# Desperodoo/distributed_multi_agent_reinforcement_learning

Hardware: AMD Instinct MI355X
Metric: env-steps/sec (whole node), pursuit-evasion 8-agent 4096-env (higher is better)
Workload: dtype f64 environment / f32 policy (f32 matrix products evaluated from exact 3-way bf16 operand splits, f32 accumulation and storage)

## Files before the change

distributed_multi_agent_reinforcement_learning_amd/csrc/mappo_split.hip:

```cpp
#include <hip/hip_runtime.h>
#include <stdint.h>
#include <string.h>

#include "mappo_ops.h"
#include "sb_gemm.hpp"
#include "sb_encoder_tail.hpp"
#include "sb_gru_seq.hpp"

extern "C" {

static int sb_gemm_any(int64_t R, int32_t N, int32_t K, const float *X, int64_t ldx, const float *W, int64_t ldw, const float *bias, int32_t relu,
                       const float *addend, int64_t lda, float *Y, int64_t ldy, uint8_t *ybits, int64_t ldyb, void *stream) {
    if (R < 0 || !X || !W || !Y || ldx < K || ldw < K || ldy < N || (addend && lda < N)) return MO_ERR_BAD_ARG;
    if ((ldx & 3) || (ldw & 3) || (ldy & 3) || (lda & 3) || ((uintptr_t)X & 15) || ((uintptr_t)W & 15) || ((uintptr_t)Y & 15) || ((uintptr_t)addend & 15) ||
        ((uintptr_t)bias & 15))
        return MO_ERR_BAD_ARG;
    if (R == 0) return 0;
    hipStream_t st = (hipStream_t)stream;
    if (N == 128 && K == 128) return launch_sb_gemm_best<4, 1>(R, X, ldx, W, ldw, bias, addend, lda, Y, ldy, relu, st, ybits, ldyb);
    if (N == 128 && K == 256) return launch_sb_gemm_best<8, 1>(R, X, ldx, W, ldw, bias, addend, lda, Y, ldy, relu, st, ybits, ldyb);
    if (ybits) return MO_ERR_BAD_ARG;
    if (N == 128 && K == 384) return launch_sb_gemm_best<12, 1>(R, X, ldx, W, ldw, bias, addend, lda, Y, ldy, relu, st);
    if (N == 256 && K == 128) return launch_sb_gemm_best<4, 2>(R, X, ldx, W, ldw, bias, addend, lda, Y, ldy, relu, st);
    if (N == 384 && K == 128) return launch_sb_gemm_best<4, 3>(R, X, ldx, W, ldw, bias, addend, lda, Y, ldy, relu, st);
    return MO_ERR_BAD_ARG;
}

int sb_gemm(int64_t R, int32_t N, int32_t K, const float *X, int64_t ldx, const float *W, int64_t ldw, const float *bias, int32_t relu,
            const float *addend, int64_t lda, float *Y, int64_t ldy, void *stream) {
// ... 41 lines not shown
    if (hipGetDevice(&dev) == hipSuccess && hipDeviceGetAttribute(&cus, hipDeviceAttributeMultiprocessorCount, dev) != hipSuccess) cus = 256;
    if (cus > 512) return MO_ERR_BAD_ARG;
    float *part = (float *)workspace;
    const float *m = (const float *)sign_bits;
    const int mt = mask_cols / 128;
    if (N == 256 && K == 128) return launch_sb_gemm<4, 2, SBG_MASK_OPT_256 | 16>(R, X, ldx, W, ldw, nullptr, m, ld_bytes, Y, ldy, 0, st, mt, part, colsum);
    if (N == 384 && K == 128) return launch_sb_gemm<4, 3, SBG_MASK_OPT_384 | 16>(R, X, ldx, W, ldw, nullptr, m, ld_bytes, Y, ldy, 0, st, mt, part, colsum);
    if (N == 128 && K == 384) return launch_sb_gemm<12, 1, SBG_MASK_OPT_K384 | 16>(R, X, ldx, W, ldw, nullptr, m, ld_bytes, Y, ldy, 0, st, mt, part, colsum);
    return MO_ERR_BAD_ARG;
}

int sb_gemm_n128(int64_t R, int32_t K, const float *X, int64_t ldx, const float *W, int64_t ldw, const float *bias, int32_t relu, const float *addend,
                 int64_t lda, float *Y, int64_t ldy, void *stream) {
    return sb_gemm(R, 128, K, X, ldx, W, ldw, bias, relu, addend, lda, Y, ldy, stream);
}

int sb_encoder_tail(int64_t Rs, const float *m3, int64_t ldx, const float *w_agg, const float *b_agg, const float *Ws, int64_t ldw, const float *C,
                    int64_t ldc, float *Y, int64_t ldy, void *stream) {
    if (Rs < 0 || !m3 || !w_agg || !b_agg || !Ws || !C || !Y || ldx < 384 || ldw < 384 || ldc < 128 || ldy < 128) return MO_ERR_BAD_ARG;
    if ((ldx & 3) || (ldw & 3) || (ldc & 3) || (ldy & 3) || ((uintptr_t)m3 & 15) || ((uintptr_t)w_agg & 15) || ((uintptr_t)b_agg & 15) || ((uintptr_t)Ws & 15) ||
        ((uintptr_t)C & 15) || ((uintptr_t)Y & 15))
        return MO_ERR_BAD_ARG;
    if (Rs == 0) return 0;
    return launch_sb_encoder_tail(Rs, m3, ldx, w_agg, b_agg, Ws, ldw, C, ldc, Y, ldy, (hipStream_t)stream);
}

int gru_seq_split_fwd_multi(int32_t n_nets, const mo_gru_seq_net *nets, int32_t T, int32_t B, int32_t H, int32_t gi_agents, void *stream) {
    if (n_nets < 1 || n_nets > MO_GRU_MAX_NETS || !nets || T < 1 || B < 1 || H != SBR_H || gi_agents < 0 || (gi_agents && B % gi_agents)) return MO_ERR_BAD_ARG;
    for (int k = 0; k < n_nets; k++) {
        const mo_gru_seq_net &m = nets[k];
        if (!m.gi || !m.w_hh || !m.b_hh || !m.h0 || !m.out) return MO_ERR_BAD_ARG;
        if ((((uintptr_t)m.gi | (uintptr_t)m.w_hh | (uintptr_t)m.b_hh | (uintptr_t)m.h0 | (uintptr_t)m.out | (uintptr_t)m.save) & 15)) return MO_ERR_BAD_ARG;
        if (m.B < 0 || m.B > B || (gi_agents && m.B % gi_agents)) return MO_ERR_BAD_ARG;
    }
    return launch_gru_seq_fwd_sb(n_nets, nets, T, B, gi_agents, (hipStream_t)stream);
}

int gru_seq_split_bwd_multi(int32_t n_nets, const mo_gru_seq_bwd_net *nets, int32_t T, int32_t B, int32_t H, int32_t gi_agents, void *stream) {
    if (n_nets < 1 || n_nets > MO_GRU_MAX_NETS || !nets || T < 1 || B < 1 || H != SBR_H || gi_agents < 0 || (gi_agents && B % gi_agents)) return MO_ERR_BAD_ARG;
    for (int k = 0; k < n_nets; k++) {
        const mo_gru_seq_bwd_net &m = nets[k];
        if (!m.dout || !m.save || !m.out || !m.h0 || !m.w_hh || !m.dgi || !m.dh0) return MO_ERR_BAD_ARG;
        if ((m.dgh == nullptr) == (m.dnr == nullptr)) return MO_ERR_BAD_ARG;
        if ((m.db_ih || m.db_hh) && (!m.db_ih || !m.db_hh || !m.workspace)) return MO_ERR_BAD_ARG;
        if ((((uintptr_t)m.dout | (uintptr_t)m.save | (uintptr_t)m.out | (uintptr_t)m.h0 | (uintptr_t)m.dgi | (uintptr_t)m.dgh | (uintptr_t)m.dnr |
              (uintptr_t)m.dh0 | (uintptr_t)m.workspace) & 15)) return MO_ERR_BAD_ARG;
        if (m.B < 0 || m.B > B || (gi_agents && m.B % gi_agents)) return MO_ERR_BAD_ARG;
// ... 6 lines not shown
```

distributed_multi_agent_reinforcement_learning_amd/csrc/sb_encoder_tail.hpp:

```cpp
#pragma once
#include <mutex>

#include "sb_common.hpp"

constexpr int SBE_IMG = 3 * 4 * 2 * 64;
constexpr int SBE_WIMG = 8 * 4 * 3 * 64;

__global__ __launch_bounds__(512) void k_sb_encoder_tail(int64_t Rs, const float *__restrict__ X, int64_t ldx, const float *__restrict__ Wa,
                                                         const float *__restrict__ ba, const float *__restrict__ Ws, int64_t ldw, const float *C,
                                                         int64_t ldc, float *Y, int64_t ldy) {
    extern __shared__ uint4 sbe_lds[];
    const int tid = threadIdx.x, w = tid >> 6, l = tid & 63, i = l & 15, gq = l >> 4;
    uint4 *const wimg = sbe_lds + w * (4 * 3 * 64) + l, *const mimg = sbe_lds + SBE_WIMG, *const eimg = mimg + SBE_IMG;
    {
        const float *rw = Wa + (size_t)(16 * w + i) * 128 + 8 * gq;
#pragma unroll
        for (int c = 0; c < 4; c++) {
            uint4 p_[3];
            sb_split8(*(const float4 *)(rw + 32 * c), *(const float4 *)(rw + 32 * c + 4), p_);
#pragma unroll
            for (int p = 0; p < 3; p++) wimg[(c * 3 + p) * 64] = p_[p];
        }
    }
    uint4 ws[12][3];
    {
        const float *rw = Ws + (size_t)(16 * w + i) * ldw + 8 * gq;
#pragma unroll
        for (int c = 0; c < 12; c++) sb_split8(*(const float4 *)(rw + 32 * c), *(const float4 *)(rw + 32 * c + 4), ws[c]);
    }
    const float4 b4 = *(const float4 *)(ba + 16 * w + 4 * gq);
    const int64_t n_t = (Rs + 31) / 32, G = gridDim.x;
    float4 pf[2];
    auto fetch = [&](int64_t t, int r) {
        const int64_t row = t * 32 + (w & 1) * 16 + i;
        pf[0] = pf[1] = make_float4(0.f, 0.f, 0.f, 0.f);
        if (row < Rs) {
            const float *src = X + row * ldx + 128 * r + 32 * (w >> 1) + 8 * gq;
            pf[0] = *(const float4 *)src;
            pf[1] = *(const float4 *)(src + 4);
        }
    };
    auto stage = [&]() {
        uint4 p_[3];
        sb_split8(pf[0], pf[1], p_);
#pragma unroll
        for (int p = 0; p < 3; p++) mimg[(p * 8 + w) * 64 + l] = p_[p];
    };
    uint2 *const edst = (uint2 *)eimg + (((w >> 1) * 2) * 64 + ((2 * (w & 1) + (gq >> 1)) << 4) + i) * 2 + (gq & 1);
    int64_t t = blockIdx.x;
    if (t < n_t) { fetch(t, 0); stage(); fetch(t, 1); }
    lds_barrier();
    for (; t < n_t; t += G) {
        const bool more = t + G < n_t;
        float4 a4[2];
#pragma unroll
        for (int rt = 0; rt < 2; rt++) {
            const int64_t row = t * 32 + rt * 16 + i;
            a4[rt] = row < Rs ? *(const float4 *)(C + row * ldc + 16 * w + 4 * gq) : make_float4(0.f, 0.f, 0.f, 0.f);
        }
        f32x4 acc_s[2];
        acc_s[0] = acc_s[1] = (f32x4){0.f, 0.f, 0.f, 0.f};
#pragma unroll
        for (int r = 0; r < 3; r++) {
            f32x4 acc_a[2];
            acc_a[0] = acc_a[1] = (f32x4){0.f, 0.f, 0.f, 0.f};
#define SBE_MMA(A, pi, pj)                                                                                                                          \
            acc[0] = __builtin_amdgcn_mfma_f32_16x16x32_bf16(__builtin_bit_cast(bf16x8, A[pi]), __builtin_bit_cast(bf16x8, b0[pj]), acc[0], 0, 0, 0); \
            acc[1] = __builtin_amdgcn_mfma_f32_16x16x32_bf16(__builtin_bit_cast(bf16x8, A[pi]), __builtin_bit_cast(bf16x8, b1[pj]), acc[1], 0, 0, 0);
#define SBE_MMA6(A) SBE_MMA(A, 2, 0) SBE_MMA(A, 0, 2) SBE_MMA(A, 1, 1) SBE_MMA(A, 1, 0) SBE_MMA(A, 0, 1) SBE_MMA(A, 0, 0)
#pragma unroll
            for (int c = 0; c < 4; c++) {
                uint4 a_[3], b0[3], b1[3];
#pragma unroll
                for (int p = 0; p < 3; p++) { a_[p] = wimg[(c * 3 + p) * 64]; b0[p] = mimg[(p * 8 + 2 * c) * 64 + l]; b1[p] = mimg[(p * 8 + 2 * c + 1) * 64 + l]; }
                f32x4(&acc)[2] = acc_a;
                SBE_MMA6(a_)
            }
#pragma unroll
            for (int rt = 0; rt < 2; rt++) {
                float4 v = make_float4(acc_a[rt][0] + b4.x, acc_a[rt][1] + b4.y, acc_a[rt][2] + b4.z, acc_a[rt][3] + b4.w);
                v.x = fmaxf(v.x, 0.f); v.y = fmaxf(v.y, 0.f); v.z = fmaxf(v.z, 0.f); v.w = fmaxf(v.w, 0.f);
                uint32_t lo[3], hi[3];
                sb_split2(v.x, v.y, lo[0], lo[1], lo[2]);
                sb_split2(v.z, v.w, hi[0], hi[1], hi[2]);
#pragma unroll
                for (int p = 0; p < 3; p++) edst[p * 8 * 64 * 2 + rt * 128] = make_uint2(lo[p], hi[p]);
            }
            lds_barrier();
            auto next_step = [&]() {
                if (r < 2 || more) stage();
                if (r == 0) fetch(t, 2);
                else if (more) fetch(t + G, r - 1);
            };
            if (w < 4) next_step();
#pragma unroll
            for (int c = 0; c < 4; c++) {
                uint4 b0[3], b1[3];
#pragma unroll
                for (int p = 0; p < 3; p++) { b0[p] = eimg[(p * 8 + 2 * c) * 64 + l]; b1[p] = eimg[(p * 8 + 2 * c + 1) * 64 + l]; }
                f32x4(&acc)[2] = acc_s;
                SBE_MMA6(ws[4 * r + c])
            }
#undef SBE_MMA6
#undef SBE_MMA
            if (w >= 4) next_step();
            if (r < 2) lds_barrier();
        }
#pragma unroll
        for (int rt = 0; rt < 2; rt++) {
            const int64_t row = t * 32 + rt * 16 + i;
            if (row < Rs) {
                float4 v = make_float4(acc_s[rt][0] + 0.f, acc_s[rt][1] + 0.f, acc_s[rt][2] + 0.f, acc_s[rt][3] + 0.f);
                v.x += a4[rt].x; v.y += a4[rt].y; v.z += a4[rt].z; v.w += a4[rt].w;
                *(float4 *)(Y + row * ldy + 16 * w + 4 * gq) = v;
            }
        }
        lds_barrier();
    }
}

inline int launch_sb_encoder_tail(int64_t Rs, const float *X, int64_t ldx, const float *Wa, const float *ba, const float *Ws, int64_t ldw,
                                  const float *C, int64_t ldc, float *Y, int64_t ldy, hipStream_t st) {
    constexpr int lds = (SBE_WIMG + 2 * SBE_IMG) * 16;
    static std::once_flag once;
    static hipError_t attr_rc = hipSuccess;
    std::call_once(once, [] { attr_rc = hipFuncSetAttribute((const void *)k_sb_encoder_tail, hipFuncAttributeMaxDynamicSharedMemorySize, lds); });
    if (attr_rc != hipSuccess) return (int)attr_rc;
    int dev = 0, cus = 256;
    if (hipGetDevice(&dev) == hipSuccess && hipDeviceGetAttribute(&cus, hipDeviceAttributeMultiprocessorCount, dev) != hipSuccess) cus = 256;
    const int64_t n_t = (Rs + 31) / 32;
    const int grid = n_t < (int64_t)cus ? (int)n_t : cus;
    hipLaunchKernelGGL(k_sb_encoder_tail, dim3(grid), dim3(512), lds, st, Rs, X, ldx, Wa, ba, Ws, ldw, C, ldc, Y, ldy);
    return (int)hipGetLastError();
}
```

distributed_multi_agent_reinforcement_learning_amd/model.py:

```python
import torch
import torch.nn as nn
import torch.nn.functional as F
from torch.nn.utils import spectral_norm
from torch.nn.utils.spectral_norm import SpectralNorm

from . import ops


class HeadLinear(nn.Linear):

    def forward(self, x):
        return ops.linear_skinny(x, self.weight, self.bias)


def _ortho_linear(n_in, n_out, cls=nn.Linear):
    layer = cls(n_in, n_out)
    for name, param in layer.named_parameters():
        if "bias" in name:
            nn.init.constant_(param, 0)
        elif "weight" in name:
            nn.init.orthogonal_(param, gain=1.0)
    return layer


# ... 17 lines not shown
        if self.num_relation != 3:
            raise NotImplementedError("num_relation must be 3 (defender, evader, obstacle)")
        self.input_dim, self.embedding_dim = input_dim, embedding_dim
        E = embedding_dim
        self.semantic_layer = _make_linear(3 * E + input_dim, E, is_sn)
        for r in range(self.num_relation):
            self.MSG_layers.append(_make_linear(2 * input_dim if r == 0 else input_dim, E, is_sn))
        for _ in range(self.depth):
            self.FCRA_layers.append(_make_linear(2 * E, E, is_sn))
        self.AGG_layers["AGG_vertex_0"] = _make_linear(E, E, is_sn)
        for k in range(self.depth):
            self.AGG_layers[f"AGG_fcra_{k}"] = _make_linear(E, E, is_sn)

    def encoder(self, p, e, o, adj_p, adj_e, adj_o, is_critic, o_kvalid=None, q_div=1, out=None, e_ref=None):
        M = self.MSG_layers
        m3 = ops.msg_agg3(p, e, o, adj_p, adj_e, adj_o, M[0].weight, M[0].bias, M[1].weight, M[1].bias, M[2].weight, M[2].bias,
                          is_critic, o_kvalid, q_div, e_ref)
        return self._after_messages(p, m3, out)

    def _after_messages(self, p, m3, out=None):
        R, P = p.shape[0], p.shape[1]
        E, ind = self.embedding_dim, self.input_dim
        agg0 = self.AGG_layers["AGG_vertex_0"]
        link = ops.ReluLink()
        emb = ops.linear(m3, agg0.weight, agg0.bias, relu=True, y_link=link)
        Ws = self.semantic_layer.weight
        p2, e2 = p.reshape(R * P, ind), emb.reshape(R * P, 3 * E)
        if out is not None:
            o2 = out.view(R * P, E)
            torch.addmm(self.semantic_layer.bias, p2, Ws[:, :ind].t(), out=o2)
            h0 = o2.addmm_(e2, Ws[:, ind:].t())
        else:
            h0 = ops.linear(e2, Ws[:, ind:], ops.linear_skinny(p2, Ws[:, :ind], self.semantic_layer.bias), consume_addend=True, x_link=link)
        return h0.reshape(R, P, E)

    def encoder_pair_train(self, p, e, o, adj_p, adj_e, adj_o, q_div=1, e_ref=None):
        M = self.MSG_layers
        m3a, m3c = ops.msg_agg3_pair_train(p, e, o, adj_p, adj_e, adj_o, M[0].weight, M[0].bias, M[1].weight, M[1].bias, M[2].weight, M[2].bias,
                                           q_div, e_ref)
        return self._after_messages(p, m3a), self._after_messages(p, m3c)

    def fcra(self, h0, hist, adj_p, is_critic, out=None):
        if self.depth == 0:
            return h0
        h, carry = h0, None
        for k in range(self.depth):
            aggk, fk = self.AGG_layers[f"AGG_fcra_{k}"], self.FCRA_layers[k]
            nb = ops.fcra_mean(z_critic=hist[k]) if is_critic else ops.fcra_mean(z_actor=hist[k], adj=adj_p)
            last = k == self.depth - 1
            h, carry = ops.fcra_hop(nb, h, carry, aggk.weight, aggk.bias, fk.weight, fk.bias, last, out if last else None)
        h.relu_link = carry[1]
        return h

    def forward(self, p, e, o, adj_p, adj_e, adj_o, hist, is_critic, o_kvalid=None, q_div=1, out=None, e_ref=None):
        h0 = self.encoder(p, e, o, adj_p, adj_e, adj_o, is_critic, o_kvalid, q_div, out if self.depth == 0 else None, e_ref)
        return self.fcra(h0, hist, adj_p, is_critic, out)
# ... 287 lines not shown
```

distributed_multi_agent_reinforcement_learning_amd/ops.py:

```python
import ctypes as C
import os

import torch
import torch.nn.functional as F

from . import build as _build

ADJ_TENSOR, ADJ_ONES, ADJ_VALID, ADJ_BITS = 0, 1, 2, 3
EXPORTS = ("dhgn_msg_agg_fwd", "dhgn_msg_agg3_fwd", "dhgn_msg_agg_bwd", "dhgn_msg_agg_bwd_workspace", "dhgn_msg_agg_ones_sorted_ok", "dhgn_msg_agg_ones_sorted_fwd",
           "dhgn_msg_agg_ones_sorted_bwd", "dhgn_msg_agg_ones_sorted_workspace", "gae_advnorm", "gae_advnorm_workspace", "categorical_sample",
           "categorical_sample_counter",
           "gru_gates_fwd", "gru_gates_bwd", "gru_cell_fwd", "gru_cell_fwd_multi", "gru_cell_split_fwd_multi", "sb_gemm_n128", "sb_gemm", "sb_encoder_tail", "gru_seq_fwd", "gru_seq_fwd_multi", "gru_seq_split_fwd_multi", "gru_seq_split_bwd_multi", "gru_seq_save_elems", "gru_seq_bwd", "gru_seq_bwd_multi", "gru_seq_bwd_workspace", "wgrad_tn", "wgrad_tn_workspace", "wgrad_split_tn", "wgrad_split_tn2", "wgrad_split_workspace", "rollout_record", "ppo_loss_fwd_bwd", "ppo_loss_prob_fwd_bwd", "ppo_loss_workspace",
           "gauss_head_sample", "ppo_loss_gauss_fwd_bwd", "ppo_loss_gauss_workspace", "gauss_head_sample_ex", "ppo_loss_gauss_ex_fwd_bwd",
           "ppo_loss_gauss_ex_workspace", "gae_advnorm_vn", "gae_advnorm_vn_workspace", "value_norm_update", "value_norm_targets",
           "ppo_loss_fwd_bwd_diag", "ppo_loss_prob_fwd_bwd_diag", "ppo_loss_gauss_fwd_bwd_diag", "ppo_loss_gauss_ex_fwd_bwd_diag",
           "ppo_loss_diag_workspace", "ppo_loss_gauss_diag_workspace", "ppo_ratio", "ppo_diag_rows_host", "fused_adam_workspace",
           "fused_adam_grid", "fused_adam_norm", "fused_adam_step", "fused_adam_advance_host", "fused_adam_rows_host", "bc_loss_workspace",
           "bc_loss_gauss_fwd_bwd", "bc_loss_gauss_ex_fwd_bwd", "bc_loss_cat_fwd_bwd", "e3d_bc_select", "n2n_bc_select", "ppo_bc_loss_workspace",
           "ppo_bc_loss_gauss_fwd_bwd", "ppo_bc_loss_cat_fwd_bwd", "mappo_ops_error_string")

_lib = None


def lib_path():
# ... 24 lines not shown
        L.dhgn_msg_agg_ones_sorted_workspace.restype = i64
        L.dhgn_msg_agg_ones_sorted_fwd.argtypes = [i32, i32, i32, i32, vp, i64, vp, i64, i32, vp, vp, vp, i64, vp, vp, vp]
        L.dhgn_msg_agg_ones_sorted_bwd.argtypes = [i32, i32, i32, i32, vp, i64, i32, vp, i64, vp, vp, vp, vp, vp, vp]
        L.gae_advnorm.argtypes = [i32, i32, i32, vp, vp, vp, f32, f32, i32, vp, vp, vp, vp]
        L.gae_advnorm_workspace.restype = i64
        L.gae_advnorm_vn.argtypes = [i32, i32, i32, vp, vp, vp, vp, vp, f32, f32, i32, vp, vp, vp, vp, vp]
        L.gae_advnorm_vn_workspace.restype = i64
        L.value_norm_update.argtypes = [vp, vp, C.c_double, vp]
        L.value_norm_targets.argtypes = [i64, vp, vp, vp, vp, vp]
        L.categorical_sample.argtypes = [i32, i32, vp, C.c_uint64, C.c_uint64, i32, vp, vp, vp]
        L.categorical_sample_counter.argtypes = [i32, i32, vp, C.c_uint64, vp, i32, vp, vp, vp]
        L.head_linear.argtypes = [i32, i32, i32, vp, vp, vp, vp, vp]
        L.head_sample.argtypes = [i32, i32, i32, vp, vp, vp, C.c_uint64, vp, vp, i32, vp, vp, vp]
        L.gru_gates_fwd.argtypes = [i32, i32, vp, vp, vp, vp, vp, vp, vp]
        L.gru_gates_bwd.argtypes = [i32, i32, vp, vp, vp, vp, vp, vp, vp, vp]
        L.gru_cell_fwd.argtypes = [i32, i32, vp, vp, vp, vp, vp, vp, vp, vp]
        L.gru_seq_fwd.argtypes = [i32, i32, i32, vp, vp, vp, vp, vp, vp, i32, vp]
        L.gru_seq_bwd.argtypes = [i32, i32, i32, vp, vp, vp, vp, vp, vp, vp, vp, vp, vp, vp, i32, vp, vp]
        L.gru_cell_fwd_multi.argtypes = [i32, vp, i32, i32, vp]
        L.gru_cell_split_fwd_multi.argtypes = [i32, vp, i32, i32, vp]
        L.sb_gemm_n128.argtypes = [i64, i32, vp, i64, vp, i64, vp, i32, vp, i64, vp, i64, vp]
        L.sb_gemm.argtypes = [i64, i32, i32, vp, i64, vp, i64, vp, i32, vp, i64, vp, i64, vp]
        L.sb_encoder_tail.argtypes = [i64, vp, i64, vp, vp, vp, i64, vp, i64, vp, i64, vp]
        L.gru_seq_fwd_multi.argtypes = [i32, vp, i32, i32, i32, i32, vp]
        L.gru_seq_bwd_multi.argtypes = [i32, vp, i32, i32, i32, i32, vp]
        L.gru_seq_split_fwd_multi.argtypes = [i32, vp, i32, i32, i32, i32, vp]
        L.gru_seq_split_bwd_multi.argtypes = [i32, vp, i32, i32, i32, i32, vp]
        L.gru_seq_save_elems.argtypes = [i32, i32]
        L.gru_seq_save_elems.restype = i64
        L.gru_seq_bwd_workspace.argtypes = [i32]
        L.gru_seq_bwd_workspace.restype = i64
        L.wgrad_tn_workspace.argtypes = [i32, i32]
        L.wgrad_tn_workspace.restype = i64
        L.wgrad_tn.argtypes = [i64, i32, i32, vp, i64, vp, i64, vp, i32, vp, vp]
        L.wgrad_split_workspace.restype = i64
        L.wgrad_split_workspace.argtypes = [i32, i32]
        L.wgrad_split_tn.argtypes = [i64, i32, i32, vp, i64, vp, i64, vp, i32, vp, vp]
        L.wgrad_split_tn2.argtypes = [i64, i32, i32, i32, vp, i64, vp, i64, vp, i64, vp, i32, vp, vp]
        L.fcra_neighbour_mean.argtypes = [i32, i32, i32, i32, vp, i64, i64, vp, i64, i64, vp, i64, vp, i32, vp, vp, i64, vp]
        L.fcra_neighbour_mean_multi.argtypes = [i32, vp, i32, i32, i32, i32, i64, i64, i64, i64, vp, i64, i32, i64, vp]
        L.sb_gemm_signs.argtypes = [i64, i32, i32, vp, i64, vp, i64, vp, i32, vp, i64, vp, i64, vp, i64, vp]
        L.sb_gemm_masked_bits.argtypes = [i64, i32, i32, vp, i64, vp, i64, vp, i64, i32, vp, i64, vp, vp, vp]
        L.sb_gemm_masked_workspace.argtypes = [i32]
        L.sb_gemm_masked_workspace.restype = i64
        L.sb_gemm_masked.argtypes = [i64, i32, i32, vp, i64, vp, i64, vp, i64, i32, vp, i64, vp, vp, vp]
        L.relu_bwd_colsum_workspace.argtypes = [i32]
# ... 1719 lines not shown
    if m3.dim() != 2 or out.dim() != 2 or m3.shape[1] != 384 or tuple(out.shape) != (m3.shape[0], 128) or tuple(Ws.shape) != (128, 384):
        return False
    if tuple(w_agg.shape) != (128, 128) or not w_agg.is_contiguous() or b_agg is None or tuple(b_agg.shape) != (128,) or not b_agg.is_contiguous():
        return False
    for t in (m3, w_agg, Ws, out):
        if t.dtype != torch.float32 or t.stride(1) != 1 or t.stride(0) % 4 or t.data_ptr() % 16:
            return False
    if b_agg.dtype != torch.float32 or b_agg.data_ptr() % 16:
        return False
    return not _overlap(m3, out)


def encoder_tail(m3, w_agg, b_agg, Ws, out):
    L = load_library()
    _check(L.sb_encoder_tail(m3.shape[0], _ptr(m3), m3.stride(0), _ptr(w_agg.detach()), _ptr(b_agg.detach()), _ptr(Ws.detach()), Ws.stride(0),
                             _ptr(out), out.stride(0), _ptr(out), out.stride(0), _stream()), "sb_encoder_tail")
    return out


def sign_bits_ok(N, K):
    return RELU_LINK and RELU_BITS and N == 128 and K in (128, 256)


PROJ_MODE = os.environ.get("MAPPO_PROJ", MATMUL_MODE)


def gru_input_projection(x2, w_ih, b_ih):
    if x2.stride(-1) == 1 and split_linear_ok(x2, w_ih, mode=PROJ_MODE, shapes=UPDATE_SPLIT_SHAPES):
        return split_linear(x2, w_ih, b_ih)
    return torch.addmm(b_ih, x2, w_ih.t())


def gru_step_multi(xs, hiddens, modules, hiddens_out=None):
    n = len(xs)
    B = xs[0].shape[0]
    outs_h = hiddens if hiddens_out is None else hiddens_out
    ok = (not torch.is_grad_enabled() and n <= 4 and B >= FUSED_CELL_MIN_ROWS and all(x.shape == (B, 128) and x.is_cuda for x in xs)
          and all(h.is_contiguous() and h.shape[1:] == (B, 128) for h in list(hiddens) + list(outs_h))
          and all(m.num_layers == modules[0].num_layers and m.weight_hh_l0.shape == (384, 128) and m.weight_ih_l0.shape == (384, 128) for m in modules))
    if not ok:
        outs = []
        for x, h, ho, m in zip(xs, hiddens, outs_h, modules):
            out, hn = gru(x.unsqueeze(0), h, m, inplace_hidden=hiddens_out is None)
            if hn is not ho:
                ho.copy_(hn)
            outs.append(ho[-1])
# ... 197 lines not shown
```

include/mappo_ops.h:

```cpp
#ifndef MAPPO_OPS_H
#define MAPPO_OPS_H
#include <stdint.h>

#ifdef __cplusplus
extern "C" {
#endif

#define MO_ERR_BAD_ARG 20001

enum { MO_ADJ_TENSOR = 0,
       MO_ADJ_ONES = 1,
       MO_ADJ_VALID = 2,
       MO_ADJ_BITS = 3 };
#define MO_ADJ_ROW_WORDS(K) (((((K) + 31) >> 5) + 3) & ~3)

int dhgn_msg_agg_fwd(int32_t R, int32_t P, int32_t K, int32_t E, int32_t din, const float *p, int64_t p_row_stride,
                     const float *q, int64_t q_row_stride, int32_t q_div, const float *e, int64_t e_row_stride, const void *adj,
                     int64_t adj_row_stride, int32_t adj_mode, const int32_t *kvalid, const float *W, const float *b,
                     float *out, int64_t out_stride , void *stream);

typedef struct mo_msg_rel {
    int32_t K, din, q_div, adj_mode;
    const float *q; int64_t q_rs;
    const float *e; int64_t e_rs;
// ... 88 lines not shown
int64_t gru_seq_bwd_workspace(int32_t B);
int gru_seq_bwd(int32_t T, int32_t B, int32_t H, const float *dout, const float *save, const float *out, const float *h0,
                const float *w_hh, float *dgi, float *dgh, float *dnr, float *dh0, float *db_ih, float *db_hh, int32_t gi_agents,
                void *workspace, void *stream);

int gru_cell_fwd(int32_t B, int32_t H, const float *x, const float *h_prev, const float *w_ih, const float *w_hh, const float *b_ih,
                 const float *b_hh, float *h_out, void *stream);
typedef struct mo_gru_cell_net { const float *x, *h_prev, *w_ih, *w_hh, *b_ih, *b_hh; float *h_out; } mo_gru_cell_net;
int gru_cell_fwd_multi(int32_t n_nets, const mo_gru_cell_net *nets, int32_t B, int32_t H, void *stream);
int gru_cell_split_fwd_multi(int32_t n_nets, const mo_gru_cell_net *nets, int32_t B, int32_t H, void *stream);
int sb_gemm_n128(int64_t R, int32_t K, const float *X, int64_t ldx, const float *W, int64_t ldw, const float *bias, int32_t relu, const float *C,
                 int64_t ldc, float *Y, int64_t ldy, void *stream);
int sb_gemm(int64_t R, int32_t N, int32_t K, const float *X, int64_t ldx, const float *W, int64_t ldw, const float *bias, int32_t relu, const float *C,
            int64_t ldc, float *Y, int64_t ldy, void *stream);
int sb_encoder_tail(int64_t Rs, const float *m3, int64_t ldx, const float *w_agg, const float *b_agg, const float *Ws, int64_t ldw, const float *C,
                    int64_t ldc, float *Y, int64_t ldy, void *stream);
int sb_gemm_signs(int64_t R, int32_t N, int32_t K, const float *X, int64_t ldx, const float *W, int64_t ldw, const float *bias, int32_t relu, const float *C,
                  int64_t ldc, float *Y, int64_t ldy, uint8_t *y_sign_bits, int64_t ld_bytes, void *stream);
int64_t sb_gemm_masked_workspace(int32_t N);
int sb_gemm_masked(int64_t R, int32_t N, int32_t K, const float *X, int64_t ldx, const float *W, int64_t ldw, const float *M, int64_t ldm,
                   int32_t mask_cols, float *Y, int64_t ldy, float *colsum, void *workspace, void *stream);
int sb_gemm_masked_bits(int64_t R, int32_t N, int32_t K, const float *X, int64_t ldx, const float *W, int64_t ldw, const uint8_t *sign_bits,
                        int64_t ld_bytes, int32_t mask_cols, float *Y, int64_t ldy, float *colsum, void *workspace, void *stream);

int64_t ppo_loss_workspace(void);
int ppo_loss_fwd_bwd(int64_t n, const float *logp_now, const float *entropy, const float *logp_old, const float *adv, const float *active,
                     const float *values_now, const float *values_old, const float *v_target, const float *active_sum, float epsilon,
                     float entropy_coef, int32_t use_value_clip, float *losses, float *grad_logp, float *grad_entropy, float *grad_values,
                     void *workspace, void *stream);
int ppo_loss_prob_fwd_bwd(int64_t n, int32_t A, const float *prob, float *grad_prob, int64_t d1, int64_t d2, int64_t p_s0, int64_t p_s1, int64_t p_s2,
                          const float *action, const float *logp_old, const float *adv, const float *active, const float *values_now, int64_t v_s0,
                          int64_t v_s1, int64_t v_s2, const float *values_old, const float *v_target, const float *active_sum, float epsilon,
                          float entropy_coef, int32_t use_value_clip, float *losses, float *grad_values, void *workspace, void *stream);

int gauss_head_sample(int32_t R, int32_t A, int32_t H, const float *feat, const float *W, const float *b, const float *log_std, uint64_t seed,
                      uint64_t *counter, uint32_t *ticket, int32_t greedy, float *action, double *env_action, float *logp, void *stream);
int64_t ppo_loss_gauss_workspace(void);
int ppo_loss_gauss_fwd_bwd(int64_t n, int32_t A, const float *mu, float *grad_mu, int64_t d1, int64_t d2, int64_t m_s0, int64_t m_s1, int64_t m_s2,
                           const float *log_std, const float *action, const float *logp_old, const float *adv, const float *active,
                           const float *values_now, int64_t v_s0, int64_t v_s1, int64_t v_s2, const float *values_old, const float *v_target,
                           const float *active_sum, float epsilon, float entropy_coef, int32_t use_value_clip, float *losses, float *grad_values,
                           float *grad_log_std, void *workspace, void *stream);

int gauss_head_sample_ex(int32_t R, int32_t A, int32_t H, const float *feat, const float *W, const float *b, const float *W_ls, const float *b_ls,
                         const float *log_std, float log_std_min, float log_std_max, int32_t squash, uint64_t seed, uint64_t *counter,
                         uint32_t *ticket, int32_t greedy, float *action, double *env_action, float *logp, void *stream);
// ... 110 lines not shown
```

Measured before the change: 2.676 million.

## Fuse encoder tail forward and backward into single training kernels

Adds a training variant of the fused encoder-tail kernel that also saves the ReLU embedding and its sign bits, plus a new fused backward kernel. The backward computes the masked gradient through the semantic weights and the aggregation layer in one pass, with per-block column sums for the bias gradient. It replaces separate linear/ReLU/linear autograd steps on the training path and is meant to cut kernel launches and intermediate memory traffic. The cost is extra stores of emb and bits in the forward and more code complexity. It only activates for large contiguous inputs in split_bf16 mode.

```diff
diff --git a/distributed_multi_agent_reinforcement_learning_amd/csrc/mappo_split.hip b/distributed_multi_agent_reinforcement_learning_amd/csrc/mappo_split.hip
--- a/distributed_multi_agent_reinforcement_learning_amd/csrc/mappo_split.hip
+++ b/distributed_multi_agent_reinforcement_learning_amd/csrc/mappo_split.hip
@@ -5,6 +5,7 @@
 #include "mappo_ops.h"
 #include "sb_gemm.hpp"
 #include "sb_encoder_tail.hpp"
+#include "sb_encoder_tail_bwd.hpp"
 #include "sb_gru_seq.hpp"
 
 extern "C" {
@@ -92,7 +93,37 @@
         ((uintptr_t)C & 15) || ((uintptr_t)Y & 15))
         return MO_ERR_BAD_ARG;
     if (Rs == 0) return 0;
-    return launch_sb_encoder_tail(Rs, m3, ldx, w_agg, b_agg, Ws, ldw, C, ldc, Y, ldy, (hipStream_t)stream);
+    return launch_sb_encoder_tail<false>(Rs, m3, ldx, w_agg, b_agg, Ws, ldw, C, ldc, Y, ldy, (hipStream_t)stream);
+}
+
+int sb_encoder_tail_train(int64_t Rs, const float *m3, int64_t ldx, const float *w_agg, const float *b_agg, const float *Ws, int64_t ldw, const float *C,
+                          int64_t ldc, float *Y, int64_t ldy, float *emb, int64_t lde, uint8_t *emb_sign_bits, int64_t ld_bytes, void *stream) {
+    if (Rs < 0 || !m3 || !w_agg || !b_agg || !Ws || !C || !Y || !emb || !emb_sign_bits || ldx < 384 || ldw < 384 || ldc < 128 || ldy < 128 || lde < 384 ||
+        ld_bytes < 48)
+        return MO_ERR_BAD_ARG;
+    if ((ldx & 3) || (ldw & 3) || (ldc & 3) || (ldy & 3) || (lde & 3) || ((uintptr_t)m3 & 15) || ((uintptr_t)w_agg & 15) || ((uintptr_t)b_agg & 15) ||
+        ((uintptr_t)Ws & 15) || ((uintptr_t)C & 15) || ((uintptr_t)Y & 15) || ((uintptr_t)emb & 15))
+        return MO_ERR_BAD_ARG;
+    if (Rs == 0) return 0;
+    return launch_sb_encoder_tail<true>(Rs, m3, ldx, w_agg, b_agg, Ws, ldw, C, ldc, Y, ldy, (hipStream_t)stream, emb, lde, emb_sign_bits, ld_bytes);
+}
+
+int64_t sb_encoder_tail_bwd_workspace(void) { return (int64_t)1024 * 384 * 4; }
+
+int sb_encoder_tail_bwd(int64_t Rs, const float *g, int64_t ldg, const float *Ws, int64_t ldw, const float *w_agg, const uint8_t *emb_sign_bits,
+                        int64_t ld_bytes, float *ga, int64_t ldga, float *d_m3, int64_t ldd, float *colsum, void *workspace, void *stream) {
+    if (Rs < 0 || !g || !Ws || !w_agg || !emb_sign_bits || !ga || !d_m3 || !colsum || !workspace || ldg < 128 || ldw < 384 || ld_bytes < 48 || ldga < 384 ||
+        ldd < 384)
+        return MO_ERR_BAD_ARG;
+    if ((ldg & 3) || (ldw & 3) || (ldga & 3) || (ldd & 3) || ((uintptr_t)g & 15) || ((uintptr_t)Ws & 15) || ((uintptr_t)w_agg & 15) || ((uintptr_t)ga & 15) ||
+        ((uintptr_t)d_m3 & 15) || ((uintptr_t)colsum & 15) || ((uintptr_t)workspace & 15))
+        return MO_ERR_BAD_ARG;
+    hipStream_t st = (hipStream_t)stream;
+    if (Rs == 0) return (int)hipMemsetAsync(colsum, 0, (size_t)384 * 4, st);
+    int dev = 0, cus = 256;
+    if (hipGetDevice(&dev) == hipSuccess && hipDeviceGetAttribute(&cus, hipDeviceAttributeMultiprocessorCount, dev) != hipSuccess) cus = 256;
+    if (cus > 1024) return MO_ERR_BAD_ARG;
+    return launch_sb_encoder_tail_bwd(Rs, g, ldg, Ws, ldw, w_agg, emb_sign_bits, ld_bytes, ga, ldga, d_m3, ldd, (float *)workspace, colsum, cus, st);
 }
 
 int gru_seq_split_fwd_multi(int32_t n_nets, const mo_gru_seq_net *nets, int32_t T, int32_t B, int32_t H, int32_t gi_agents, void *stream) {
diff --git a/distributed_multi_agent_reinforcement_learning_amd/csrc/sb_encoder_tail.hpp b/distributed_multi_agent_reinforcement_learning_amd/csrc/sb_encoder_tail.hpp
--- a/distributed_multi_agent_reinforcement_learning_amd/csrc/sb_encoder_tail.hpp
+++ b/distributed_multi_agent_reinforcement_learning_amd/csrc/sb_encoder_tail.hpp
@@ -6,9 +6,11 @@
 constexpr int SBE_IMG = 3 * 4 * 2 * 64;
 constexpr int SBE_WIMG = 8 * 4 * 3 * 64;
 
+template <bool SAVE>
 __global__ __launch_bounds__(512) void k_sb_encoder_tail(int64_t Rs, const float *__restrict__ X, int64_t ldx, const float *__restrict__ Wa,
                                                          const float *__restrict__ ba, const float *__restrict__ Ws, int64_t ldw, const float *C,
-                                                         int64_t ldc, float *Y, int64_t ldy) {
+                                                         int64_t ldc, float *Y, int64_t ldy, float *__restrict__ emb, int64_t lde,
+                                                         uint8_t *__restrict__ ebits, int64_t ldb) {
     extern __shared__ uint4 sbe_lds[];
     const int tid = threadIdx.x, w = tid >> 6, l = tid & 63, i = l & 15, gq = l >> 4;
     uint4 *const wimg = sbe_lds + w * (4 * 3 * 64) + l, *const mimg = sbe_lds + SBE_WIMG, *const eimg = mimg + SBE_IMG;
@@ -53,11 +55,14 @@
     for (; t < n_t; t += G) {
         const bool more = t + G < n_t;
         float4 a4[2];
+        auto addend = [&]() {
 #pragma unroll
-        for (int rt = 0; rt < 2; rt++) {
-            const int64_t row = t * 32 + rt * 16 + i;
-            a4[rt] = row < Rs ? *(const float4 *)(C + row * ldc + 16 * w + 4 * gq) : make_float4(0.f, 0.f, 0.f, 0.f);
-        }
+            for (int rt = 0; rt < 2; rt++) {
+                const int64_t row = t * 32 + rt * 16 + i;
+                a4[rt] = row < Rs ? *(const float4 *)(C + row * ldc + 16 * w + 4 * gq) : make_float4(0.f, 0.f, 0.f, 0.f);
+            }
+        };
+        if constexpr (!SAVE) addend();
         f32x4 acc_s[2];
         acc_s[0] = acc_s[1] = (f32x4){0.f, 0.f, 0.f, 0.f};
 #pragma unroll
@@ -80,6 +85,15 @@
             for (int rt = 0; rt < 2; rt++) {
                 float4 v = make_float4(acc_a[rt][0] + b4.x, acc_a[rt][1] + b4.y, acc_a[rt][2] + b4.z, acc_a[rt][3] + b4.w);
                 v.x = fmaxf(v.x, 0.f); v.y = fmaxf(v.y, 0.f); v.z = fmaxf(v.z, 0.f); v.w = fmaxf(v.w, 0.f);
+                if constexpr (SAVE) {
+                    const int64_t row = t * 32 + rt * 16 + i;
+                    const unsigned nib = (unsigned)(v.x > 0.f) | ((unsigned)(v.y > 0.f) << 1) | ((unsigned)(v.z > 0.f) << 2) | ((unsigned)(v.w > 0.f) << 3);
+                    const unsigned other = (unsigned)__shfl_xor((int)nib, 16);
+                    if (row < Rs) {
+                        *(float4 *)(emb + row * lde + 128 * r + 16 * w + 4 * gq) = v;
+                        if (!(gq & 1)) ebits[row * ldb + 16 * r + 2 * w + (gq >> 1)] = (uint8_t)(nib | (other << 4));
+                    }
+                }
                 uint32_t lo[3], hi[3];
                 sb_split2(v.x, v.y, lo[0], lo[1], lo[2]);
                 sb_split2(v.z, v.w, hi[0], hi[1], hi[2]);
@@ -87,6 +101,7 @@
                 for (int p = 0; p < 3; p++) edst[p * 8 * 64 * 2 + rt * 128] = make_uint2(lo[p], hi[p]);
             }
             lds_barrier();
+            if constexpr (SAVE) if (r == 2) addend();
             auto next_step = [&]() {
                 if (r < 2 || more) stage();
                 if (r == 0) fetch(t, 2);
@@ -119,17 +134,19 @@
     }
 }
 
-inline int launch_sb_encoder_tail(int64_t Rs, const float *X, int64_t ldx, const float *Wa, const float *ba, const float *Ws, int64_t ldw,
-                                  const float *C, int64_t ldc, float *Y, int64_t ldy, hipStream_t st) {
+template <bool SAVE = false>
+int launch_sb_encoder_tail(int64_t Rs, const float *X, int64_t ldx, const float *Wa, const float *ba, const float *Ws, int64_t ldw, const float *C,
+                           int64_t ldc, float *Y, int64_t ldy, hipStream_t st, float *emb = nullptr, int64_t lde = 0, uint8_t *ebits = nullptr,
+                           int64_t ldb = 0) {
     constexpr int lds = (SBE_WIMG + 2 * SBE_IMG) * 16;
     static std::once_flag once;
     static hipError_t attr_rc = hipSuccess;
-    std::call_once(once, [] { attr_rc = hipFuncSetAttribute((const void *)k_sb_encoder_tail, hipFuncAttributeMaxDynamicSharedMemorySize, lds); });
+    std::call_once(once, [] { attr_rc = hipFuncSetAttribute((const void *)k_sb_encoder_tail<SAVE>, hipFuncAttributeMaxDynamicSharedMemorySize, lds); });
     if (attr_rc != hipSuccess) return (int)attr_rc;
     int dev = 0, cus = 256;
     if (hipGetDevice(&dev) == hipSuccess && hipDeviceGetAttribute(&cus, hipDeviceAttributeMultiprocessorCount, dev) != hipSuccess) cus = 256;
     const int64_t n_t = (Rs + 31) / 32;
     const int grid = n_t < (int64_t)cus ? (int)n_t : cus;
-    hipLaunchKernelGGL(k_sb_encoder_tail, dim3(grid), dim3(512), lds, st, Rs, X, ldx, Wa, ba, Ws, ldw, C, ldc, Y, ldy);
+    hipLaunchKernelGGL(k_sb_encoder_tail<SAVE>, dim3(grid), dim3(512), lds, st, Rs, X, ldx, Wa, ba, Ws, ldw, C, ldc, Y, ldy, emb, lde, ebits, ldb);
     return (int)hipGetLastError();
 }
diff --git a/distributed_multi_agent_reinforcement_learning_amd/csrc/sb_encoder_tail_bwd.hpp b/distributed_multi_agent_reinforcement_learning_amd/csrc/sb_encoder_tail_bwd.hpp
--- /dev/null
+++ b/distributed_multi_agent_reinforcement_learning_amd/csrc/sb_encoder_tail_bwd.hpp
@@ -0,0 +1,157 @@
+#pragma once
+#include <mutex>
+
+#include "sb_common.hpp"
+#include "sb_encoder_tail.hpp"
+#include "sb_gemm.hpp"
+
+__global__ __launch_bounds__(512) void k_sb_encoder_tail_bwd(int64_t Rs, const float *__restrict__ G, int64_t ldg, const float *__restrict__ Ws,
+                                                             int64_t ldw, const float *__restrict__ Wa, const uint8_t *__restrict__ ebits, int64_t ldb,
+                                                             float *__restrict__ GA, int64_t ldga, float *__restrict__ DM, int64_t ldd,
+                                                             float *__restrict__ colsum_part) {
+    extern __shared__ uint4 sbe_lds[];
+    const int tid = threadIdx.x, w = tid >> 6, l = tid & 63, i = l & 15, gq = l >> 4;
+    uint4 *const wimg = sbe_lds + w * (4 * 3 * 64) + l, *const gimg = sbe_lds + SBE_WIMG, *const aimg = gimg + SBE_IMG;
+    {
+        const float *cw = Wa + (size_t)(8 * gq) * 128 + 16 * w + i;
+#pragma unroll
+        for (int c = 0; c < 4; c++) {
+            const float *s = cw + (size_t)(32 * c) * 128;
+            uint4 p_[3];
+            sb_split8(make_float4(s[0], s[128], s[256], s[384]), make_float4(s[512], s[640], s[768], s[896]), p_);
+#pragma unroll
+            for (int p = 0; p < 3; p++) wimg[(c * 3 + p) * 64] = p_[p];
+        }
+    }
+    uint4 ws[12][3];
+    {
+        const float *cw = Ws + (size_t)(8 * gq) * ldw + 16 * w + i;
+#pragma unroll
+        for (int r = 0; r < 3; r++) {
+#pragma unroll
+            for (int c = 0; c < 4; c++) {
+                const float *s = cw + (size_t)(32 * c) * ldw + 128 * r;
+                sb_split8(make_float4(s[0], s[ldw], s[2 * ldw], s[3 * ldw]), make_float4(s[4 * ldw], s[5 * ldw], s[6 * ldw], s[7 * ldw]), ws[4 * r + c]);
+            }
+        }
+    }
+    const int64_t n_t = (Rs + 31) / 32, G_ = gridDim.x;
+    float4 pf[2];
+    auto fetch = [&](int64_t t) {
+        const int64_t row = t * 32 + (w & 1) * 16 + i;
+        pf[0] = pf[1] = make_float4(0.f, 0.f, 0.f, 0.f);
+        if (row < Rs) {
+            const float *src = G + row * ldg + 32 * (w >> 1) + 8 * gq;
+            pf[0] = *(const float4 *)src;
+            pf[1] = *(const float4 *)(src + 4);
+        }
+    };
+    auto stage = [&]() {
+        uint4 p_[3];
+        sb_split8(pf[0], pf[1], p_);
+#pragma unroll
+        for (int p = 0; p < 3; p++) gimg[(p * 8 + w) * 64 + l] = p_[p];
+    };
+    uint2 *const adst = (uint2 *)aimg + (((w >> 1) * 2) * 64 + ((2 * (w & 1) + (gq >> 1)) << 4) + i) * 2 + (gq & 1);
+    float4 cs[3];
+#pragma unroll
+    for (int r = 0; r < 3; r++) cs[r] = make_float4(0.f, 0.f, 0.f, 0.f);
+    unsigned mbn[2];
+    auto mask = [&](int64_t t, int r) {
+#pragma unroll
+        for (int rt = 0; rt < 2; rt++) {
+            const int64_t row = t * 32 + rt * 16 + i;
+            mbn[rt] = row < Rs ? (unsigned)ebits[row * ldb + 16 * r + 2 * w + (gq >> 1)] : 255u;
+        }
+    };
+    int64_t t = blockIdx.x;
+    if (t < n_t) { fetch(t); stage(); mask(t, 0); }
+    if (t + G_ < n_t) fetch(t + G_);
+    lds_barrier();
+    for (; t < n_t; t += G_) {
+        const bool more = t + G_ < n_t;
+#pragma unroll
+        for (int r = 0; r < 3; r++) {
+            unsigned mb[2] = {mbn[0], mbn[1]};
+            if (r < 2) mask(t, r + 1);
+            else if (more) mask(t + G_, 0);
+            f32x4 acc[2];
+            acc[0] = acc[1] = (f32x4){0.f, 0.f, 0.f, 0.f};
+#define SBE_MMA(A, pi, pj)                                                                                                                          \
+            acc[0] = __builtin_amdgcn_mfma_f32_16x16x32_bf16(__builtin_bit_cast(bf16x8, A[pi]), __builtin_bit_cast(bf16x8, b0[pj]), acc[0], 0, 0, 0); \
+            acc[1] = __builtin_amdgcn_mfma_f32_16x16x32_bf16(__builtin_bit_cast(bf16x8, A[pi]), __builtin_bit_cast(bf16x8, b1[pj]), acc[1], 0, 0, 0);
+#define SBE_MMA6(A) SBE_MMA(A, 2, 0) SBE_MMA(A, 0, 2) SBE_MMA(A, 1, 1) SBE_MMA(A, 1, 0) SBE_MMA(A, 0, 1) SBE_MMA(A, 0, 0)
+#pragma unroll
+            for (int c = 0; c < 4; c++) {
+                uint4 b0[3], b1[3];
+#pragma unroll
+                for (int p = 0; p < 3; p++) { b0[p] = gimg[(p * 8 + 2 * c) * 64 + l]; b1[p] = gimg[(p * 8 + 2 * c + 1) * 64 + l]; }
+                SBE_MMA6(ws[4 * r + c])
+            }
+#pragma unroll
+            for (int rt = 0; rt < 2; rt++) {
+                const int64_t row = t * 32 + rt * 16 + i;
+                const unsigned m = mb[rt] >> ((gq & 1) * 4);
+                float4 v = make_float4(acc[rt][0], acc[rt][1], acc[rt][2], acc[rt][3]);
+                v.x = (m & 1u) ? v.x : 0.f; v.y = (m & 2u) ? v.y : 0.f; v.z = (m & 4u) ? v.z : 0.f; v.w = (m & 8u) ? v.w : 0.f;
+                if (row < Rs) {
+                    cs[r].x += v.x; cs[r].y += v.y; cs[r].z += v.z; cs[r].w += v.w;
+                    *(float4 *)(GA + row * ldga + 128 * r + 16 * w + 4 * gq) = v;
+                }
+                uint32_t lo[3], hi[3];
+                sb_split2(v.x, v.y, lo[0], lo[1], lo[2]);
+                sb_split2(v.z, v.w, hi[0], hi[1], hi[2]);
+#pragma unroll
+                for (int p = 0; p < 3; p++) adst[p * 8 * 64 * 2 + rt * 128] = make_uint2(lo[p], hi[p]);
+            }
+            lds_barrier();
+            auto next_tile = [&]() {
+                if (more) stage();
+                if (t + 2 * G_ < n_t) fetch(t + 2 * G_);
+            };
+            if (r == 2 && w < 4) next_tile();
+            acc[0] = acc[1] = (f32x4){0.f, 0.f, 0.f, 0.f};
+#pragma unroll
+            for (int c = 0; c < 4; c++) {
+                uint4 a_[3], b0[3], b1[3];
+#pragma unroll
+                for (int p = 0; p < 3; p++) { a_[p] = wimg[(c * 3 + p) * 64]; b0[p] = aimg[(p * 8 + 2 * c) * 64 + l]; b1[p] = aimg[(p * 8 + 2 * c + 1) * 64 + l]; }
+                SBE_MMA6(a_)
+            }
+#undef SBE_MMA6
+#undef SBE_MMA
+            if (r == 2 && w >= 4) next_tile();
+#pragma unroll
+            for (int rt = 0; rt < 2; rt++) {
+                const int64_t row = t * 32 + rt * 16 + i;
+                if (row < Rs)
+                    *(float4 *)(DM + row * ldd + 128 * r + 16 * w + 4 * gq) = make_float4(acc[rt][0] + 0.f, acc[rt][1] + 0.f, acc[rt][2] + 0.f, acc[rt][3] + 0.f);
+            }
+            lds_barrier();
+        }
+    }
+#pragma unroll
+    for (int r = 0; r < 3; r++) {
+#pragma unroll
+        for (int m = 1; m < 16; m <<= 1) {
+            cs[r].x += __shfl_xor(cs[r].x, m); cs[r].y += __shfl_xor(cs[r].y, m);
+            cs[r].z += __shfl_xor(cs[r].z, m); cs[r].w += __shfl_xor(cs[r].w, m);
+        }
+        if (i == 0) *(float4 *)(colsum_part + (size_t)blockIdx.x * 384 + 128 * r + 16 * w + 4 * gq) = cs[r];
+    }
+}
+
+inline int launch_sb_encoder_tail_bwd(int64_t Rs, const float *G, int64_t ldg, const float *Ws, int64_t ldw, const float *Wa, const uint8_t *ebits,
+                                      int64_t ldb, float *GA, int64_t ldga, float *DM, int64_t ldd, float *colsum_part, float *colsum, int cus,
+                                      hipStream_t st) {
+    constexpr int lds = (SBE_WIMG + 2 * SBE_IMG) * 16;
+    static std::once_flag once;
+    static hipError_t attr_rc = hipSuccess;
+    std::call_once(once, [] { attr_rc = hipFuncSetAttribute((const void *)k_sb_encoder_tail_bwd, hipFuncAttributeMaxDynamicSharedMemorySize, lds); });
+    if (attr_rc != hipSuccess) return (int)attr_rc;
+    const int64_t n_t = (Rs + 31) / 32;
+    const int grid = n_t < (int64_t)cus ? (int)n_t : cus;
+    hipLaunchKernelGGL(k_sb_encoder_tail_bwd, dim3(grid), dim3(512), lds, st, Rs, G, ldg, Ws, ldw, Wa, ebits, ldb, GA, ldga, DM, ldd, colsum_part);
+    hipLaunchKernelGGL(k_sb_colsum_reduce, dim3(3), dim3(128), 0, st, grid, 384, colsum_part, colsum);
+    return (int)hipGetLastError();
+}
diff --git a/distributed_multi_agent_reinforcement_learning_amd/model.py b/distributed_multi_agent_reinforcement_learning_amd/model.py
--- a/distributed_multi_agent_reinforcement_learning_amd/model.py
+++ b/distributed_multi_agent_reinforcement_learning_amd/model.py
@@ -63,16 +63,24 @@
         R, P = p.shape[0], p.shape[1]
         E, ind = self.embedding_dim, self.input_dim
         agg0 = self.AGG_layers["AGG_vertex_0"]
+        Ws = self.semantic_layer.weight
+        pos = None
+        if out is None and ops.ENCODER_TAIL_TRAIN and torch.is_grad_enabled() and m3.is_contiguous():
+            pos = ops.linear_skinny(p.reshape(R * P, ind), Ws[:, :ind], self.semantic_layer.bias)
+            m3_s, Wse = m3.view(R * P, 3 * E), Ws[:, ind:]
+            if pos.requires_grad and ops.encoder_tail_train_ok(m3_s, agg0.weight, agg0.bias, Wse, pos):
+                return ops.encoder_tail_train(m3_s, agg0.weight, agg0.bias, Wse, pos).reshape(R, P, E)
         link = ops.ReluLink()
         emb = ops.linear(m3, agg0.weight, agg0.bias, relu=True, y_link=link)
-        Ws = self.semantic_layer.weight
         p2, e2 = p.reshape(R * P, ind), emb.reshape(R * P, 3 * E)
         if out is not None:
             o2 = out.view(R * P, E)
             torch.addmm(self.semantic_layer.bias, p2, Ws[:, :ind].t(), out=o2)
             h0 = o2.addmm_(e2, Ws[:, ind:].t())
         else:
-            h0 = ops.linear(e2, Ws[:, ind:], ops.linear_skinny(p2, Ws[:, :ind], self.semantic_layer.bias), consume_addend=True, x_link=link)
+            if pos is None:
+                pos = ops.linear_skinny(p2, Ws[:, :ind], self.semantic_layer.bias)
+            h0 = ops.linear(e2, Ws[:, ind:], pos, consume_addend=True, x_link=link)
         return h0.reshape(R, P, E)
 
     def encoder_pair_train(self, p, e, o, adj_p, adj_e, adj_o, q_div=1, e_ref=None):
diff --git a/distributed_multi_agent_reinforcement_learning_amd/ops.py b/distributed_multi_agent_reinforcement_learning_amd/ops.py
--- a/distributed_multi_agent_reinforcement_learning_amd/ops.py
+++ b/distributed_multi_agent_reinforcement_learning_amd/ops.py
@@ -70,6 +70,10 @@
         L.sb_gemm_n128.argtypes = [i64, i32, vp, i64, vp, i64, vp, i32, vp, i64, vp, i64, vp]
         L.sb_gemm.argtypes = [i64, i32, i32, vp, i64, vp, i64, vp, i32, vp, i64, vp, i64, vp]
         L.sb_encoder_tail.argtypes = [i64, vp, i64, vp, vp, vp, i64, vp, i64, vp, i64, vp]
+        L.sb_encoder_tail_train.argtypes = [i64, vp, i64, vp, vp, vp, i64, vp, i64, vp, i64, vp, i64, vp, i64, vp]
+        L.sb_encoder_tail_bwd_workspace.argtypes = []
+        L.sb_encoder_tail_bwd_workspace.restype = i64
+        L.sb_encoder_tail_bwd.argtypes = [i64, vp, i64, vp, i64, vp, vp, i64, vp, i64, vp, i64, vp, vp, vp]
         L.gru_seq_fwd_multi.argtypes = [i32, vp, i32, i32, i32, i32, vp]
         L.gru_seq_bwd_multi.argtypes = [i32, vp, i32, i32, i32, i32, vp]
         L.gru_seq_split_fwd_multi.argtypes = [i32, vp, i32, i32, i32, i32, vp]
@@ -1835,6 +1839,76 @@
     return RELU_LINK and RELU_BITS and N == 128 and K in (128, 256)
 
 
+ENCODER_TAIL_TRAIN = os.environ.get("MAPPO_ENCODER_TAIL_TRAIN", "1") != "0"
+ENCODER_TAIL_TRAIN_MIN_ROWS = 32768
+
+
+def encoder_tail_train_ok(m3, w_agg, b_agg, Ws, addend):
+    if not ENCODER_TAIL_TRAIN or PROJ_MODE != "split_bf16" or not (RELU_LINK and RELU_BITS) or not m3.is_cuda:
+        return False
+    if m3.dim() != 2 or addend.dim() != 2 or m3.shape[1] != 384 or tuple(addend.shape) != (m3.shape[0], 128) or tuple(Ws.shape) != (128, 384):
+        return False
+    if m3.shape[0] < ENCODER_TAIL_TRAIN_MIN_ROWS or not m3.is_contiguous() or not addend.is_contiguous():
+        return False
+    if tuple(w_agg.shape) != (128, 128) or not w_agg.is_contiguous() or b_agg is None or tuple(b_agg.shape) != (128,) or not b_agg.is_contiguous():
+        return False
+    for t in (m3, w_agg, Ws, addend):
+        if t.dtype != torch.float32 or t.stride(1) != 1 or t.stride(0) % 4 or t.data_ptr() % 16:
+            return False
+    if b_agg.dtype != torch.float32 or b_agg.data_ptr() % 16:
+        return False
+    return not _overlap(m3, addend)
+
+
+def encoder_tail_train_fwd(m3, w_agg, b_agg, Ws, C, Y, emb, bits):
+    L = load_library()
+    _check(L.sb_encoder_tail_train(m3.shape[0], _ptr(m3), m3.stride(0), _ptr(w_agg.detach()), _ptr(b_agg.detach()), _ptr(Ws.detach()), Ws.stride(0),
+                                   _ptr(C), C.stride(0), _ptr(Y), Y.stride(0), _ptr(emb), emb.stride(0), _ptr(bits), bits.stride(0), _stream()),
+           "sb_encoder_tail_train")
+    return Y
+
+
+def encoder_tail_train_bwd(g, Ws, w_agg, bits):
+    L = load_library()
+    Rs = g.shape[0]
+    ga = torch.empty((Rs, 384), dtype=torch.float32, device=g.device)
+    d_m3 = torch.empty((Rs, 384), dtype=torch.float32, device=g.device)
+    cs = torch.empty(384, dtype=torch.float32, device=g.device)
+    ws = torch.empty(L.sb_encoder_tail_bwd_workspace(), dtype=torch.uint8, device=g.device)
+    _check(L.sb_encoder_tail_bwd(Rs, _ptr(g), g.stride(0), _ptr(Ws.detach()), Ws.stride(0), _ptr(w_agg.detach()), _ptr(bits), bits.stride(0), _ptr(ga),
+                                 ga.stride(0), _ptr(d_m3), d_m3.stride(0), _ptr(cs), _ptr(ws), _stream()), "sb_encoder_tail_bwd")
+    return ga, d_m3, cs
+
+
+class _EncoderTailTrain(torch.autograd.Function):
+
+    @staticmethod
+    def forward(ctx, m3, w_agg, b_agg, Ws, addend):
+        Rs = m3.shape[0]
+        emb = torch.empty((Rs, 384), dtype=torch.float32, device=m3.device)
+        bits = torch.empty((Rs, 48), dtype=torch.uint8, device=m3.device)
+        ctx.mark_dirty(addend)
+        encoder_tail_train_fwd(m3, w_agg, b_agg, Ws, addend, addend, emb, bits)
+        ctx.save_for_backward(m3, emb, bits, w_agg, Ws)
+        return addend
+
+    @staticmethod
+    def backward(ctx, g):
+        m3, emb, bits, w_agg, Ws = ctx.saved_tensors
+        g2 = g.reshape(-1, 128)
+        if g2.stride(1) != 1 or g2.stride(0) % 4 or g2.data_ptr() % 16:
+            g2 = g2.contiguous()
+        ga, d_m3, cs = encoder_tail_train_bwd(g2, Ws, w_agg, bits)
+        dWs = wgrad(g2, emb) if ctx.needs_input_grad[3] else None
+        dWa = wgrad(ga.view(-1, 128), m3.view(-1, 128)) if ctx.needs_input_grad[1] else None
+        db = cs.view(-1, 128).sum(0) if ctx.needs_input_grad[2] else None
+        return (d_m3 if ctx.needs_input_grad[0] else None), dWa, db, dWs, (g if ctx.needs_input_grad[4] else None)
+
+
+def encoder_tail_train(m3, w_agg, b_agg, Ws, addend):
+    return _EncoderTailTrain.apply(m3, w_agg, b_agg, Ws, addend)
+
+
 PROJ_MODE = os.environ.get("MAPPO_PROJ", MATMUL_MODE)
 
 
diff --git a/include/mappo_ops.h b/include/mappo_ops.h
--- a/include/mappo_ops.h
+++ b/include/mappo_ops.h
@@ -134,6 +134,11 @@
                    int32_t mask_cols, float *Y, int64_t ldy, float *colsum, void *workspace, void *stream);
 int sb_gemm_masked_bits(int64_t R, int32_t N, int32_t K, const float *X, int64_t ldx, const float *W, int64_t ldw, const uint8_t *sign_bits,
                         int64_t ld_bytes, int32_t mask_cols, float *Y, int64_t ldy, float *colsum, void *workspace, void *stream);
+int sb_encoder_tail_train(int64_t Rs, const float *m3, int64_t ldx, const float *w_agg, const float *b_agg, const float *Ws, int64_t ldw, const float *C,
+                          int64_t ldc, float *Y, int64_t ldy, float *emb, int64_t lde, uint8_t *emb_sign_bits, int64_t ld_bytes, void *stream);
+int64_t sb_encoder_tail_bwd_workspace(void);
+int sb_encoder_tail_bwd(int64_t Rs, const float *g, int64_t ldg, const float *Ws, int64_t ldw, const float *w_agg, const uint8_t *emb_sign_bits,
+                        int64_t ld_bytes, float *ga, int64_t ldga, float *d_m3, int64_t ldd, float *colsum, void *workspace, void *stream);
 
 int64_t ppo_loss_workspace(void);
 int ppo_loss_fwd_bwd(int64_t n, const float *logp_now, const float *entropy, const float *logp_old, const float *adv, const float *active,
```

After: 2.729 million, median of 6. 1.02x the previous value.
